# MichaelAxtmann/InPlaceMSDradixsort

Measured on AMD Instinct MI355X. Metric: Gkeys/s + achieved HBM GB/s, 2^30 uniform u32 keys, 1/2/4/8 MI355X, higher is better.
Workload: dtype u32; 1 GPU; 2^30 uniform u32 keys per GPU, in-place MSD radix sort, 8-bit digits; config_id=c2, elements_per_gpu=1073741824, steps_verified=0, verified_by=not checked in a plain run (bench.py --full verifies every timed step), workspace_bytes=360054784

## Files before the change

inplacemsdradixsort_amd/csrc/msd_device.hpp:

```cpp
#pragma once

#include <hip/hip_runtime.h>
#include <stdint.h>

namespace msd {

constexpr int kP = 256;
constexpr uint32_t kXBase = 0x80000000u;
constexpr uint32_t kNoOwner = 0xFFFFFFFFu;
constexpr uint32_t kRposStride = 32;

struct NoVal {};
typedef uint32_t u32x4 __attribute__((ext_vector_type(4)));

template <typename V> struct has_val { static constexpr bool value = true; };
template <> struct has_val<NoVal> { static constexpr bool value = false; };

template <typename K, typename V> struct Cfg;
template <> struct Cfg<uint32_t, NoVal> {
	static constexpr int B = 64, T = 4096, TH = 1024;
	static constexpr int SORT_TH = 1024, SORT_KPT = 24;
};
template <> struct Cfg<uint64_t, NoVal> {
	static constexpr int B = 32, T = 4096, TH = 1024;
// ... 317 lines not shown
	}
#pragma unroll
	for (int o = 32; o > 0; o >>= 1) {
		seen += (uint32_t)__shfl_xor((int)seen, o);
		same += (uint32_t)__shfl_xor((int)same, o);
	}
	if ((tid & 63) == 0 && seen) {
		atomicAdd(&plans[st.parent].adj_seen, seen);
		atomicAdd(&plans[st.parent].adj_same, same);
	}
}

#ifndef MSD_UNEVEN_PCT
#define MSD_UNEVEN_PCT 125
#endif
__device__ __forceinline__ bool direct_declines(uint32_t mn, uint32_t mx, uint32_t adj_same, uint32_t adj_seen)
{
	const bool runs = (uint64_t)adj_same * 8u > adj_seen;
	return runs || !(mn > 0 && (double)mx * 100.0 <= (double)MSD_UNEVEN_PCT * (double)mn);
}

template <int B>
__global__ __launch_bounds__(256) void direct_plan_kernel(const Parent *__restrict__ parents, DirectPlan *__restrict__ plans,
	Counters *__restrict__ ctr)
{
	__shared__ uint64_t tmp[8];
	__shared__ uint32_t s_mn, s_mx;
	const Parent pa = parents[blockIdx.x];
	DirectPlan *plan = plans + blockIdx.x;
	const uint32_t d = threadIdx.x;
	if (d == 0) {
		s_mn = 0xFFFFFFFFu;
		s_mx = 0;
	}
	const uint64_t s0 = (pa.start + B - 1) / B, s1 = (pa.start + pa.count) / B;
	uint64_t total;
	const uint64_t c = plan->est_cnt[d];
	const uint64_t ex = block_excl_scan256_64(c, tmp, total);
	const uint64_t ns = s1 > s0 ? s1 - s0 : 0;
	plan->bound[d] = (uint32_t)(s0 + (total ? ex * ns / total : (uint64_t)d * ns / kP));
	if (d == 0) plan->bound[kP] = (uint32_t)s1;
	if (d < (1u << pa.width)) {
		atomicMin(&s_mn, (uint32_t)c);
		atomicMax(&s_mx, (uint32_t)c);
	}
	__syncthreads();
	if (d == 0 && direct_declines(s_mn, s_mx, plan->adj_same, plan->adj_seen)) atomicAdd(&ctr->direct_uneven, 1u);
}

__device__ __forceinline__ bool wave_select_smallest(uint32_t v, bool elig, int need, uint64_t &mask_out)
{
	uint64_t cand = __ballot(elig), selm = 0;
	if ((int)__popcll(cand) > need) {
#pragma unroll
		for (int bit = 9; bit >= 0; --bit) {
			const uint64_t zeros = cand & ~__ballot((v >> bit) & 1u);
// ... 1950 lines not shown
```

inplacemsdradixsort_amd/csrc/msd_front16.hpp:

```cpp
#pragma once

namespace msd {

constexpr int kF16Th = 1024;
constexpr uint32_t kF16Words = 1u << 15;
constexpr size_t kF16Lds = (size_t)kF16Words * 4 + 64 * 4;
constexpr int kF16Loads = 8;

struct FrontSummary {
	uint32_t top[kP];
	unsigned long long v_or, v_and;
	uint32_t adj_seen, adj_same[2];
	uint32_t overflow;
	uint32_t uneven[2];
	uint32_t nroute[5];
	uint32_t hopeless;
};
static_assert(sizeof(FrontSummary) % 8 == 0, "the OR / AND words take 64-bit atomics");

__device__ __forceinline__ void front_clear(FrontSummary *__restrict__ sum)
{
	uint32_t *w = reinterpret_cast<uint32_t *>(sum);
	for (uint32_t i = threadIdx.x; i < sizeof(FrontSummary) / 4; i += blockDim.x) w[i] = 0;
	__syncthreads();
	if (threadIdx.x == 0) sum->v_and = ~0ull;
}
__global__ __launch_bounds__(256) void front_init_kernel(FrontSummary *__restrict__ sum) { front_clear(sum); }

constexpr int kFpRuns = 32;
template <typename K>
__global__ __launch_bounds__(1024) void front_probe_kernel(const K *__restrict__ keys, uint64_t n, uint32_t shift, FrontSummary *__restrict__ sum)
{
	__shared__ uint32_t h[kP], s_mn, s_mx, s_same;
	const uint32_t tid = threadIdx.x;
	if (tid < kP) h[tid] = 0;
	if (tid == 0) {
		s_mn = 0xFFFFFFFFu;
		s_mx = 0;
		s_same = 0;
// ... 133 lines not shown
{
	__shared__ uint32_t s_st[3], s_r[5];
	if (sum->hopeless) return;
	const uint32_t t = threadIdx.x, p = blockIdx.x * kP + t, sh = (p & 1u) * 16u;
	if (t == 0) {
		s_st[0] = 0xFFFFFFFFu;
		s_st[1] = 0;
		s_st[2] = 0;
	}
	if (t < 5) s_r[t] = 0;
	__syncthreads();
	const uint32_t *src = partials + (p >> 1);
	uint32_t c = 0;
#pragma unroll 8
	for (uint32_t w = 0; w < nparts; ++w) c += (src[(size_t)w * kF16Words] >> sh) & 0xFFFFu;
	hist[p] = c;
	atomicAdd(&s_r[(int)route_child(c, child_bits, stop_bits, count_bits, small_max, med_max, true) + 1], 1u);
	front_row_stats(c, s_st);
	if (t == 0) {
		sum->top[blockIdx.x] = s_st[2];
		if (direct_declines(s_st[0], s_st[1], sum->adj_same[1], sum->adj_seen)) atomicAdd(&sum->uneven[1], 1u);
	}
	if (t < 5 && s_r[t]) atomicAdd(&sum->nroute[t], s_r[t]);
}

__global__ __launch_bounds__(256) void front_top_kernel(FrontSummary *__restrict__ sum)
{
	__shared__ uint32_t s_st[3];
	if (sum->hopeless) return;
	if (threadIdx.x == 0) {
		s_st[0] = 0xFFFFFFFFu;
		s_st[1] = 0;
		s_st[2] = 0;
	}
	__syncthreads();
	front_row_stats(sum->top[threadIdx.x], s_st);
	if (threadIdx.x == 0 && direct_declines(s_st[0], s_st[1], sum->adj_same[0], sum->adj_seen)) sum->uneven[0] = 1;
}

__global__ __launch_bounds__(256) void front_apply_kernel(DirectPlan *__restrict__ plans, const uint32_t *__restrict__ hist,
	const FrontSummary *__restrict__ sum, uint32_t rows)
{
	DirectPlan *plan = plans + blockIdx.x;
	plan->est_cnt[threadIdx.x] = rows ? hist[blockIdx.x * kP + threadIdx.x] : sum->top[threadIdx.x];
	if (threadIdx.x == 0) {
		plan->adj_seen = sum->adj_seen;
		plan->adj_same = sum->adj_same[rows ? 1 : 0];
	}
}

}
```

inplacemsdradixsort_amd/csrc/msd_radix.hip:

```cpp
#include "msd_device.hpp"
#include "msd_select.hpp"
#include "msd_select_rows.hpp"
#include "msd_reverse.hpp"
#include "msd_sort_rows.hpp"
#include "msd_runs.hpp"
#include "msd_reduce.hpp"
#include "msd_scan.hpp"
#include "msd_compact.hpp"
#include "msd_search.hpp"
#include "msd_merge2.hpp"
#include "msd_setops.hpp"
#include "msd_join.hpp"
#include "msd_args.hpp"
#include "../../include/msd_radix_hip.h"
#include "../../include/msd_sort_keys_hip.h"
#include "../../include/msd_sort_rows_hip.h"
#include "../../include/msd_runs_hip.h"
#include "../../include/msd_reduce_hip.h"
#include "../../include/msd_scan_hip.h"
#include "../../include/msd_compact_hip.h"
#include "../../include/msd_search_hip.h"
#include "../../include/msd_merge_hip.h"
#include "../../include/msd_setops_hip.h"
#include "../../include/msd_join_hip.h"
// ... 8 lines not shown
#include <vector>

using namespace msd;

#define MSD_VERSION "inplacemsdradixsort_amd 0.2 (gfx950)"

struct PhaseRec {
	const char *name;
	hipEvent_t ev;
};

struct msd_ctx {
	int device = 0;
	hipStream_t stream = nullptr;
	char *slab = nullptr;
	size_t slab_bytes = 0;
	char *keep = nullptr;
	size_t keep_bytes = 0;
	Segment *lists = nullptr;
	size_t lists_cap = 0;
	void *pinned = nullptr;
	size_t pinned_bytes = 0;
	hipEvent_t ev_early = nullptr;
	std::string err;
	bool profiling = false;
	hipEvent_t ev_start = nullptr;
	std::vector<PhaseRec> phases;
	std::vector<hipEvent_t> ev_pool;
	size_t ev_used = 0;
	std::vector<std::pair<std::string, double>> phase_us;
	std::vector<std::pair<std::string, uint64_t>> stats;
	int sm_count = 256;
	int chains_per_cu[3] = { 4, 4, 2 };
	int direct_mode = 1;
	uint64_t direct_min = 1ull << 22;
	uint64_t direct_min_parent = 1ull << 17;
	int regpart = 1;
	int count16 = 1;
	int leaf17 = 1;
	int mid_leaf = 1;
	int early_leaves = 1;
	int early_plan = 1;
	int front_count = 1;
	uint64_t front_min = 1ull << 29;
	const uint32_t *order_keys = nullptr;
	uint64_t order_n = 0;
	int merge_leaf = 0;
	char *sel = nullptr;
	size_t sel_bytes = 0;
	uint64_t select_cap = 1ull << 20;
	int topk_rows_mode = 0;
	int topk_rows_lanes = 0;
	char *rows_stage = nullptr;
	size_t rows_stage_bytes = 0;
	int sort_rows_mode = 0;
	int sort_rows_lanes = 0;
	uint64_t *fix_plan = nullptr;
	int fix_stats = 0;
	uint64_t fix_split = 0;
	int search_mode = 0;
	uint64_t search_merge_ratio = 32;
};

static int fail(msd_ctx *c, int code, const char *fmt, ...)
{
	char buf[512];
	va_list ap;
// ... 419 lines not shown
template <typename K, typename V>
static size_t round_bytes_estimate(uint64_t n, int sm_count)
{
	using C = Cfg<K, V>;
	const uint64_t small_max = (uint64_t)C::SORT_TH * C::SORT_KPT;
	size_t worst = 0;
	for (int shape = 0; shape < 2; ++shape) {
		std::vector<Segment> segs;
		if (shape == 0)
			segs.push_back({ 0, n, (uint32_t)(sizeof(K) * 8), 0 });
		else if (n > 512 * small_max)
			for (int i = 0; i < 256; ++i) segs.push_back({ n / 256 * i, n / 256, (uint32_t)(sizeof(K) * 8 - 8), 0 });
		if (segs.empty()) continue;
		RoundPlan rp;
		plan_round<K, V>(segs, small_max, sm_count, rp);
		Bump b(nullptr);
		RoundBufs rb;
		carve_round<K, V>(b, rp, small_max, rb);
		worst = std::max(worst, b.off);
	}
	return worst + 4096;
}

template <typename K> struct SortJob {
	enum Kind {
		kWhole,
		kDigit,
		kRanges,
		kOffsets,
		kList,
	} kind = kWhole;
	uint32_t stop_bits = 0;
	unsigned shift = 0, width = 0;
	uint64_t *counts = nullptr;
	const K *splitters = nullptr;
	const uint64_t *seg_off = nullptr;
	uint32_t nsplit = 0, nseg = 0;
	const std::vector<Segment> *segs = nullptr;

	static SortJob whole(uint32_t stop_bits = 0) { return { kWhole, stop_bits }; }
	static SortJob digit(unsigned shift, unsigned width, uint64_t *counts) { return { kDigit, 0, shift, width, counts }; }
	static SortJob ranges(const K *delims, uint32_t nsplit, unsigned width, uint64_t *counts) { return { kRanges, 0, 0, width, counts, delims, nullptr, nsplit }; }
	static SortJob offsets(const uint64_t *seg_off, uint32_t nseg) { return { kOffsets, 0, 0, 0, nullptr, nullptr, seg_off, 0, nseg }; }
	static SortJob list(const std::vector<Segment> &segs) { return { kList, 0, 0, 0, nullptr, nullptr, nullptr, 0, 0, &segs }; }
	bool single_pass() const { return kind == kDigit || kind == kRanges; }
	bool segmented() const { return kind == kOffsets || kind == kList; }
// ... 101 lines not shown
			if (top_sample > 0 && c->direct_mode != 0 && n >= c->direct_min && n >= ((uint64_t)1 << 24)) {
				unverified = true;
				claimed_const = low_mask & ~(((uint64_t)1 << top_sample) - 1ull);
				cur[0].bits = (uint32_t)top_sample;
				set_stat(c, "skipped_bits", (uint64_t)(end_bit - top_sample));
			} else {
				rc = run_vary(1, &vary);
				if (rc) return rc;
				vary &= low_mask;
				const int top = vary ? 64 - __builtin_clzll(vary) : 0;
				set_stat(c, "skipped_bits", (uint64_t)(end_bit - top));
				if (top == 0)
					cur.clear();
				else
					cur[0].bits = (uint32_t)top;
			}
		}
		phase_mark(c, "bit skip");
		if (!cur.empty() && cur[0].bits <= job.stop_bits) cur.clear();
		return MSD_OK;
	}

	bool front = false;
	FrontSummary fsum;
	uint32_t *front_hist() const { return reinterpret_cast<uint32_t *>(c->lists + c->lists_cap); }
	FrontSummary *front_sum() const { return reinterpret_cast<FrontSummary *>(front_hist() + (size_t)kP * kP); }
	int front_count()
	{
		if constexpr (!HV && sizeof(K) == 4) {
			if (!c->front_count || job.kind != SortJob<K>::kWhole || job.stop_bits || end_bit != 32 || cur.size() != 1 || c->direct_mode == 0 ||
			    n < c->direct_min || n < c->front_min || n < ((uint64_t)1 << 20) || n >= ((uint64_t)1 << 32))
				return MSD_OK;
			{
				const uint64_t mean = n / kP;
				if (pick_width(n, 32, small_max, count_bits) != 8 || mean - mean / 8 < c->direct_min_parent ||
				    pick_width(mean - mean / 8, 24, small_max, count_bits) != 8 || pick_width(mean + mean / 8, 24, small_max, count_bits) != 8)
					return MSD_OK;
			}
			int rc = slab_reserve(c, round_bytes_estimate<K, V>(n, c->sm_count), true);
			if (!rc) rc = lists_reserve(c, (size_t)kP * kP + 16, 0, 0);
			if (rc) return rc;
			static_assert(((size_t)kP * kP + 16) * sizeof(Segment) >= (size_t)kP * kP * 4 + sizeof(FrontSummary), "the counts and the summary fit a quarter of the lists");
			const unsigned grid = (unsigned)std::min<uint64_t>({ (uint64_t)c->sm_count, std::max<uint64_t>(1, n >> 18), c->slab_bytes / (kF16Words * sizeof(uint32_t)) });
			if (!grid) return MSD_OK;
			uint32_t *partials = reinterpret_cast<uint32_t *>(c->slab);
			LAUNCH(c, (front_probe_kernel<K>), 1, 1024, 0, keys, n, 16u, front_sum());
			LAUNCH(c, (front_count16_kernel<K>), grid, kF16Th, kF16Lds, keys, n, 16u, partials, front_sum());
			LAUNCH(c, front_plan_kernel, kP, 256, 0, partials, grid, front_hist(), front_sum(), 16u, job.stop_bits, count_bits, small_max,
			       std::max<uint64_t>(small_max, kCountMedMax));
			LAUNCH(c, front_top_kernel, 1, 256, 0, front_sum());
			HIPCHK(c, hipMemcpyAsync(c->pinned, front_sum(), sizeof(FrontSummary), hipMemcpyDeviceToHost, c->stream));
			HIPCHK(c, hipStreamSynchronize(c->stream));
			memcpy(&fsum, c->pinned, sizeof fsum);
			phase_mark(c, "front count");
			const uint64_t vary = (fsum.v_or ^ fsum.v_and) & low_mask;
			const int top = vary ? 64 - __builtin_clzll(vary) : 0;
			if (fsum.hopeless) {
				add_stat(c, "front_count_declined", 1);
				return MSD_OK;
			}
			bool ok = !fsum.overflow && top + 8 > end_bit && !fsum.uneven[0] && !fsum.uneven[1] && fsum.nroute[kRouteCount + 1] == (uint32_t)kP * kP;
			std::vector<Segment> next = front_parents();
			uint64_t total = 0;
			for (const Segment &sg : next) {
				ok = ok && sg.count >= c->direct_min_parent && pick_width(sg.count, sg.bits, small_max, count_bits) == 8;
				total += sg.count;
			}
			if (!fsum.overflow && total != n) return fail(c, MSD_EINTERNAL, "front count: the counts add up to %llu of %llu keys", (unsigned long long)total, (unsigned long long)n);
			add_stat(c, ok ? "front_count_sorts" : "front_count_declined", 1);
			front = ok;
		}
		return MSD_OK;
	}
	std::vector<Segment> front_parents() const
	{
		std::vector<Segment> v;
		uint64_t at = 0;
		for (int d = 0; d < kP; ++d) {
			v.push_back({ at, fsum.top[d], (uint32_t)end_bit - 8u, 0 });
			at += fsum.top[d];
		}
		return v;
	}

	int route_to_leaves()
	{
		if (job.segmented() && !cur.empty()) {
			std::vector<Segment> l_small, l_count, l_big, parents;
			for (auto &sg : cur) {
				Route to = route_child(sg.count, sg.bits, job.stop_bits, HV ? 0u : count_bits, small_max, std::max<uint64_t>(small_max, kCountMedMax), !HV);
				if (to == kRouteDone) continue;
				if (to == kRouteBig && l_big.size() >= big_cap) to = kRouteNext;
// ... 32 lines not shown
		return MSD_OK;
	}

	int rounds()
	{
		while (!cur.empty() || dev_np) {
			int rc;
			if constexpr (sizeof(K) == 8) {
				if (!job.single_pass() && c->regpart) {
					std::vector<Segment> fit, rest;
					if (!dev_np)
						for (auto &sg : cur) (sg.count + 1 <= kRpCap && sg.count > small_max ? fit : rest).push_back(sg);
					if (dev_np || fit.size() >= 64 || (!fit.empty() && rest.empty())) {
						if constexpr (HV)
							rc = c->leaf17 && leaf17_ok && !unverified ? leaf17_pass(fit, rest) : regpart_round(fit, rest);
						else
							rc = regpart_round(fit, rest);
						if (rc) return rc;
						continue;
					}
				}
			}
			Round r;
			if ((rc = plan_upload(r)) || (rc = classify(r)) || (rc = permute_blocks(r)) || (rc = cleanup_collect(r)) ||
			    (rc = r.leaves_follow ? early_summary(r) : r.plan_ahead ? plan_next_early(r) : round_summary(r)))
				return rc;
		}
		return MSD_OK;
	}

	int leaf17_pass(const std::vector<Segment> &fit, const std::vector<Segment> &rest)
	{
		const bool on_device = dev_np != 0;
		const uint32_t np = on_device ? dev_np : (uint32_t)fit.size();
		dev_np = 0;
		int rc = slab_reserve(c, 2 * (size_t)np * sizeof(Segment) + 4096);
		if (!rc) rc = pinned_reserve(c, (size_t)np * sizeof(Segment) + 4096);
		if (rc) return rc;
		Segment *d_segs = reinterpret_cast<Segment *>(c->slab), *d_rej = d_segs + np;
		if (on_device)
			HIPCHK(c, hipMemcpyAsync(d_segs, dev_list, (size_t)np * sizeof(Segment), hipMemcpyDeviceToDevice, c->stream));
		else if ((rc = upload(c, { { d_segs, fit.data(), (size_t)np * sizeof(Segment) } })))
			return rc;
		HIPCHK(c, hipMemsetAsync(&ctr->nslow2, 0, sizeof(uint32_t), c->stream));
		HIPCHK(c, hipMemsetAsync(&ctr->l17_slow, 0, sizeof(uint32_t), c->stream));
		phase_mark(c, "plan+upload");
		LAUNCH(c, (leaf17_kernel<V>), std::min<uint32_t>(np, (uint32_t)c->sm_count), kL17Th, kL17Lds, keys, vals, d_segs, np, d_rej, &ctr->nslow2, ctr, 0);
// ... 63 lines not shown
		ncount_host = hc.ncount;
		nbig_host = hc.nbig;
		add_stat(c, "rounds", 1);
		add_stat(c, "regpart_rounds", 1);
		add_stat(c, "parents", np);
		add_stat(c, "children", nc);
		cur = rest;
		if (hc.next_parents && (rc = fetch_segments(c, d_next, hc.next_parents, cur, (char *)c->pinned + 256, ahead))) return rc;
		phase_mark(c, "readback");
		prev_direct = false;
		++round;
		return MSD_OK;
	}

	struct Round {
		RoundPlan rp;
		RoundBufs rb;
		uint32_t np = 0, ns = 0, nc = 0;
		bool tried_direct = false;
		bool hist_checks = false;
		bool leaves_follow = false;
		size_t plan_ahead = 0;
	};
	static constexpr size_t kReadAhead = 2048, kSegOff = 256, kVresOff = kSegOff - 2 * sizeof(unsigned long long);
	static constexpr size_t kEarlyOff = kSegOff + kReadAhead * sizeof(Segment), kStagingBytes = kEarlyOff + sizeof(Counters);
	static_assert(sizeof(Counters) <= kVresOff, "counters and the OR/AND words share the head of the staging buffer");
	static constexpr size_t kPlanCtrOff = (kStagingBytes + 255) / 256 * 256, kPlanSegOff = kPlanCtrOff + 256;
	static constexpr size_t kParkOff = kPlanSegOff + kReadAhead * sizeof(Segment), kStage2Off = (kParkOff + sizeof(Counters) + 255) / 256 * 256;
	static_assert(sizeof(Counters) <= 256, "the early copy of the counters has 256 bytes");
	struct Pending {
		bool open = false;
		int round = 0;
		uint32_t np = 0, ns = 0, nc = 0;
		uint64_t nslots = 0;
	} pending;
	Pending parked;
	bool parked_direct = false;
	bool enqueue_ahead = false;
	Counters *park() const { return ctr + 2; }
	static size_t stage2_bytes(size_t np, size_t ns) { return kStage2Off + np * sizeof(Parent) + ns * sizeof(Stripe); }
	void plan_next(const std::vector<Segment> &segs, RoundPlan &rp) const
	{
		plan_round<K, V>(segs, small_max, c->sm_count, rp, count_bits, job.single_pass() ? job.width : 0u, job.splitters ? job.nsplit : 0u);
	}
	int plan_upload(Round &r)
	{
		const bool ahead = enqueue_ahead;
		enqueue_ahead = false;
		plan_next(cur, r.rp);
		const bool first = round == 0;
		int rc = slab_carve(c, [&](Bump &b) { carve_round<K, V>(b, r.rp, small_max, r.rb); },
				    first && !job.single_pass() ? round_bytes_estimate<K, V>(n, c->sm_count) : 0, first);
		if (rc) return rc;
		r.np = (uint32_t)r.rp.parents.size(), r.ns = (uint32_t)r.rp.stripes.size(), r.nc = r.rp.nchildren;
		if constexpr (!HV) {
			r.leaves_follow = !job.single_pass() && !unverified && c->early_leaves;
			for (size_t i = 0; i < r.np && r.leaves_follow; ++i) r.leaves_follow = r.rp.parents[i].shift <= count_bits;
		}
		if ((rc = lists_reserve(c, (size_t)std::max(nsmall_host, ncount_host) + r.nc + 16, nsmall_host, ncount_host))) return rc;
		{
			static_assert(sizeof(Parent) % 4 == 0 && sizeof(Stripe) % 4 == 0, "the plan travels as 32-bit words");
			const uint64_t plan_words = (r.np <= kDirectMaxParents ? r.np : 1) * sizeof(DirectPlan) / sizeof(uint32_t);
			const uint64_t ntiles = (r.nc + kScanTile - 1) / kScanTile + 1;
			const uint64_t parent_words = r.np * sizeof(Parent) / 4, stripe_words = r.ns * sizeof(Stripe) / 4;
			const size_t next_stripes = (size_t)std::max<uint64_t>((uint64_t)c->sm_count * MSD_STRIPE_WANT, n >> MSD_STRIPE_CAP_LOG) + 2 * kReadAhead + 64;
			const size_t want = !ahead && c->early_plan && !job.single_pass() ? stage2_bytes(kReadAhead, next_stripes) : 0;
			if ((rc = pinned_reserve(c, std::max({ kStagingBytes, r.np * sizeof(Parent) + r.ns * sizeof(Stripe), want })))) return rc;
			char *stage = (char *)c->pinned + (ahead ? kStage2Off : 0);
			if (!ahead) HIPCHK(c, hipStreamSynchronize(c->stream));
			memcpy(stage, r.rp.parents.data(), r.np * sizeof(Parent));
			memcpy(stage + r.np * sizeof(Parent), r.rp.stripes.data(), r.ns * sizeof(Stripe));
			void *staged = nullptr;
			HIPCHK(c, hipHostGetDevicePointer(&staged, c->pinned, 0));
			staged = (char *)staged + (stage - (char *)c->pinned);
			const unsigned grid = (unsigned)std::min<uint64_t>(1024, (std::max({ plan_words, ntiles, parent_words, stripe_words }) + 255) / 256 + 1);
			LAUNCH(c, round_init_kernel, grid, 256, 0, ctr, reinterpret_cast<uint32_t *>(r.rb.plans), plan_words, r.rb.scan_state, ntiles, r.rb.scan_ctr,
			       static_cast<const uint32_t *>(staged), reinterpret_cast<uint32_t *>(r.rb.parents), parent_words,
			       reinterpret_cast<uint32_t *>(r.rb.stripes), stripe_words, ahead ? park() : nullptr);
		}
		phase_mark(c, "plan+upload");
		return MSD_OK;
	}

	int classify_direct(Round &r)
	{
		const RoundPlan &rp = r.rp;
		const uint32_t np = r.np, ns = r.ns;
		bool try_direct = c->direct_mode != 0 && rp.round_keys >= c->direct_min && !job.splitters;
		for (size_t i = 0; i < np && try_direct; ++i) try_direct = rp.parents[i].width == 8 || c->direct_mode == 2;
		if (try_direct && np > 1) {
			try_direct = prev_direct && np <= kDirectMaxParents;
			for (size_t i = 0; i < np && try_direct; ++i) try_direct = rp.parents[i].count >= c->direct_min_parent;
		}
		for (size_t i = 0; i < ns && try_direct; ++i)
			try_direct = rp.stripes[i].end - rp.stripes[i].begin >= (((uint64_t)1 << rp.parents[rp.stripes[i].parent].width) * (B - 1) + 2 * B);
		uint64_t max_piece = 0;
		for (size_t i = 0; i < np && try_direct; ++i)
			max_piece = std::max<uint64_t>(max_piece, rp.parents[i].count / B / (rp.parents[i].stripe_hi - rp.parents[i].stripe_lo) + 2);
		if (front && (round > 1 || np != (round == 0 ? 1u : (uint32_t)kP))) front = false;
		if (!try_direct || max_piece >= 65535) {
			front = false;
			return MSD_OK;
		}
		const RoundBufs &rb = r.rb;
		if (front) {
			LAUNCH(c, front_apply_kernel, np, 256, 0, rb.plans, front_hist(), front_sum(), (uint32_t)round);
		} else if (np == 1) {
			const uint64_t nruns = rp.parents[0].count / 256;
			const uint32_t every = (uint32_t)std::min<uint64_t>(64, std::max<uint64_t>(1, nruns / 16384));
			const uint32_t sgrid = (uint32_t)std::min<uint64_t>(1024, std::max<uint64_t>(1, nruns / every / 4));
			LAUNCH(c, (direct_sample_kernel<K>), sgrid, 256, 0, keys, rb.parents, rb.plans, every);
		} else {
			r.hist_checks = unverified && rp.round_keys == n;
			if (r.hist_checks) {
				if (int rc = vres_init()) return rc;
				add_stat(c, "bit_skip_checked_by_histogram", 1);
			}
			LAUNCH(c, (direct_hist_kernel<K>), ns, 1024, 0, keys, rb.stripes, rb.parents, rb.plans, r.hist_checks ? vres : nullptr);
		}
		LAUNCH(c, (direct_plan_kernel<B>), np, 256, 0, rb.parents, rb.plans, ctr);
		phase_mark(c, front ? "A front counts" : np == 1 ? "A sample" : "A histogram");
		r.tried_direct = true;
		const uint32_t force = c->direct_mode == 2 ? 1u : 0u;
		LAUNCH(c, (classify_direct2_kernel<K, V>), ns, (Direct2Cfg<K, V>::TH), (Direct2Lds<K, V>::bytes), keys, vals, rb.stripes, rb.parents, rb.plans,
		       block_map, slot_full, rb.fb, rb.lo_cnt, rb.lo_off, rb.lo_keys, rb.lo_vals, rb.nfull, ctr, force);
		phase_mark(c, "A classify direct");
		return MSD_OK;
	}

	int classify(Round &r)
	{
		if (int rc = classify_direct(r)) return rc;
		if (!r.tried_direct || c->direct_mode != 2) {
			const RoundBufs &rb = r.rb;
			const uint32_t *run_if = r.tried_direct ? &ctr->direct_uneven : nullptr;
			if (job.splitters)
				LAUNCH(c, (classify_stream2_kernel<K, V, true>), r.ns, (Stream2Cfg<K, V>::TH), (Stream2Lds<K, V>::range_bytes), keys, vals, rb.stripes,
				       rb.parents, block_map, rb.fb, rb.lo_cnt, rb.lo_off, rb.lo_keys, rb.lo_vals, rb.nfull, job.splitters, run_if);
			else
				LAUNCH(c, (classify_stream2_kernel<K, V, false>), r.ns, (Stream2Cfg<K, V>::TH), (Stream2Lds<K, V>::bytes), keys, vals, rb.stripes,
				       rb.parents, block_map, rb.fb, rb.lo_cnt, rb.lo_off, rb.lo_keys, rb.lo_vals, rb.nfull, nullptr, run_if);
		}
		phase_mark(c, "A classify");
// ... 30 lines not shown
		LAUNCH(c, (chains_kernel<K, V>), grid, 256, 0, rb.ca, rb.list, rb.holes, ctr, keys, vals, rb.xkeys, rb.xvals, n / B, 4 * nc + kMinChains);
		phase_mark(c, "B block permute");
		return MSD_OK;
	}

	bool may_leave_parents(const Round &r) const
	{
		uint64_t leaf_max = small_max;
		if constexpr (sizeof(K) == 8)
			if (c->regpart) leaf_max = std::max<uint64_t>(leaf_max, kRpCap - 1);
		for (const Parent &p : r.rp.parents)
			if ((p.count >> p.width) > leaf_max) return true;
		return false;
	}

	int collect(Round &r)
	{
		const RoundBufs &rb = r.rb;
		const uint32_t np = r.np, nc = r.nc;
		const bool sp = job.single_pass();
		uint32_t wmax = 1;
		for (size_t i = 0; i < np; ++i) wmax = std::max(wmax, r.rp.parents[i].width);
		const uint32_t small_cap = (uint32_t)std::min<size_t>(c->lists_cap, 0xFFFFFFFFu);
		LAUNCH(c, collect_kernel, (np + (256u >> wmax) - 1) / (256u >> wmax), 256, 0, rb.parents, np, wmax, rb.ca,
		       sp ? ~0ull : small_max, (HV || sp) ? small_max : std::max<uint64_t>(small_max, kCountMedMax),
		       small_cap, sp ? 0u : count_bits,
		       rb.next_parents, small(), small_count(), (HV || sp) ? nullptr : big, big_cap, ctr,
		       (sp && job.counts) ? job.counts : nullptr, job.splitters ? job.nsplit + 1u : nc, job.stop_bits);
		if (r.leaves_follow) {
			if (front && round == 1) return MSD_OK;
			if (!c->ev_early) HIPCHK(c, hipEventCreateWithFlags(&c->ev_early, hipEventDisableTiming));
			HIPCHK(c, hipMemcpyAsync((char *)c->pinned + kEarlyOff, ctr, sizeof(Counters), hipMemcpyDeviceToHost, c->stream));
			HIPCHK(c, hipEventRecord(c->ev_early, c->stream));
		} else if (c->early_plan && !sp && !r.hist_checks && !parked.open && c->pinned_bytes >= kStage2Off && may_leave_parents(r)) {
			r.plan_ahead = std::min<size_t>(r.rp.round_keys / (small_max + 1) + 2, kReadAhead);
			if (front && round == 0) return MSD_OK;
			if (!c->ev_early) HIPCHK(c, hipEventCreateWithFlags(&c->ev_early, hipEventDisableTiming));
			HIPCHK(c, hipMemcpyAsync((char *)c->pinned + kPlanCtrOff, ctr, sizeof(Counters), hipMemcpyDeviceToHost, c->stream));
			HIPCHK(c, hipMemcpyAsync((char *)c->pinned + kPlanSegOff, rb.next_parents, r.plan_ahead * sizeof(Segment), hipMemcpyDeviceToHost, c->stream));
			HIPCHK(c, hipEventRecord(c->ev_early, c->stream));
		}
		return MSD_OK;
	}

	int cleanup_collect(Round &r)
	{
		const RoundBufs &rb = r.rb;
// ... 124 lines not shown
			if ((h[0] ^ h[1]) & claimed_const) {
				exact_vary = h[0] ^ h[1];
				phase_mark(c, "readback");
				return kRestart;
			}
			unverified = false;
		}
		prev_direct = r.tried_direct && (hc.direct_uneven == 0 || c->direct_mode == 2);
		if (prev_direct) add_stat(c, "direct_rounds", 1);
		nsmall_host = hc.nsmall;
		ncount_host = hc.ncount;
		nbig_host = hc.nbig;
		round_stats(hc, r.np, r.ns, r.nc, r.rp.nslots);
		cur.clear();
		if (job.single_pass()) return MSD_OK;
		bool stays_on_device = false;
		if constexpr (sizeof(K) == 8) {
			if (c->regpart && hc.next_parents >= 64 && (uint64_t)hc.next_max + 1 <= kRpCap) {
				HIPCHK(c, hipMemcpyAsync(dev_list, r.rb.next_parents, (size_t)hc.next_parents * sizeof(Segment), hipMemcpyDeviceToDevice, c->stream));
				dev_np = hc.next_parents;
				stays_on_device = true;
			}
		}
		if (hc.next_parents && !stays_on_device &&
		    (rc = fetch_segments(c, r.rb.next_parents, hc.next_parents, cur, (char *)c->pinned + kSegOff, ahead)))
			return rc;
		phase_mark(c, "readback");
		++round;
		return MSD_OK;
	}

	int verify_skip()
	{
		if (!unverified) return MSD_OK;
		uint64_t vary = 0;
		if (int rc = run_vary(1, &vary)) return rc;
		phase_mark(c, "bit skip");
		if (vary & claimed_const) {
			exact_vary = vary;
			return kRestart;
		}
		unverified = false;
		return MSD_OK;
	}

	int start_over()
	{
		const uint64_t vary = exact_vary & low_mask;
		const int top = vary ? 64 - __builtin_clzll(vary) : 0;
		set_stat(c, "skipped_bits", (uint64_t)(end_bit - top));
		add_stat(c, "bit_skip_restarts", 1);
		cur.clear();
		if (top > 0 && (uint32_t)top > job.stop_bits) cur.push_back({ 0, n, (uint32_t)top, 0 });
		nsmall_host = ncount_host = nbig_host = dev_np = 0;
		round = 0;
		pending.open = parked.open = enqueue_ahead = false;
		prev_direct = unverified = front = false;
		HIPCHK(c, hipMemsetAsync(ctr, 0, sizeof(Counters), c->stream));
		return MSD_OK;
	}

	int count_leaves()
	{
		if constexpr (!HV) {
			if (!ncount_host || job.single_pass()) return MSD_OK;
			int rc = slab_reserve(c, 3 * (size_t)ncount_host * sizeof(Segment) + 4096);
			if (rc) return rc;
			Segment *slow = reinterpret_cast<Segment *>(c->slab), *rej16 = slow + ncount_host, *slow2 = rej16 + ncount_host;
			const uint32_t count_grid = std::min<uint32_t>(ncount_host, (uint32_t)c->sm_count * 2);
			const bool c16 = sizeof(K) == 4 && (c->count16 == 2 || (c->count16 == 1 && n / ncount_host >= 12000));
			if constexpr (sizeof(K) == 4)
				if (c16) LAUNCH(c, count_place16_kernel, count_grid, kC16Th, kC16Lds, keys, small_count(), ncount_host, rej16, ctr, n);
			LAUNCH(c, (count_place_kernel<K>), count_grid, kCountTh, kCountLds, keys, c16 ? rej16 : small_count(), c16 ? 0u : ncount_host,
			       c16 ? &ctr->nslow16 : nullptr, slow, ctr);
			const uint32_t *walk_n = &ctr->nslow;
			const Segment *walk_list = slow;
			if constexpr (sizeof(K) == 4) {
				if (c->mid_leaf) {
					LAUNCH(c, (merge_count_kernel<true>), std::min<uint32_t>(ncount_host, (uint32_t)c->sm_count), kMcTh, kMcLds, keys, keys, nullptr,
					       nullptr, nullptr, 0, 0, 0, 0, slow, &ctr->nslow, slow2, &ctr->nslow2, &ctr->count_ticket4, nullptr);
					walk_n = &ctr->nslow2;
					walk_list = slow2;
				}
			}
			LAUNCH(c, (count_walk_kernel<K>), count_grid, kCountTh, kCountLds, keys, walk_list, walk_n, small(), nsmall_host, small_max, big, big_cap, ctr);
			phase_mark(c, "count sort");
			Counters hc;
			if ((rc = read_counters(c, ctr, hc, { parked_piece() })) || (rc = parked_summary())) return rc;
			if (pending.open) {
				pending.open = false;
				if (hc.errors && (hc.err_sites & ~0x80u || !hc.err_sites))
					return round_errors(hc, pending.round, pending.np, pending.ns, prev_direct ? "used" : "not used");
				round_stats(hc, pending.np, pending.ns, pending.nc, pending.nslots);
			}
			if (hc.errors) return fail(c, MSD_EINTERNAL, "counting leaf: %u segments could not be queued", hc.errors);
			set_stat(c, "count16_rejected", hc.nslow16);
			set_stat(c, "count_slow_segments", hc.nslow);
			nbig_host = hc.nbig;
			nfallback_known = hc.nfallback;
		}
		return MSD_OK;
	}

	int big_count_sort()
	{
		if constexpr (!HV) {
			if (!nbig_host || job.single_pass()) return MSD_OK;
			std::vector<Segment> bs;
			int rc = fetch(c, big, nbig_host, bs);
			if (rc) return rc;
			const uint32_t batch_max = 4096;
			for (uint32_t b0 = 0; b0 < nbig_host; b0 += batch_max) {
				const uint32_t nb = std::min(batch_max, nbig_host - b0);
				constexpr uint32_t tile_elems = big_tile_elems<K>() * kBigGroup;
				std::vector<uint32_t> first(2 * ((size_t)nb + 1));
				uint32_t *first_chunk = first.data(), *first_tile = first.data() + nb + 1;
				uint64_t nchunks = 0, ntiles = 0;
				for (uint32_t i = 0; i < nb; ++i) {
					first_chunk[i] = (uint32_t)nchunks;
					first_tile[i] = (uint32_t)ntiles;
					nchunks += (bs[b0 + i].count + kBigChunk - 1) / kBigChunk;
					ntiles += (bs[b0 + i].count + tile_elems - 1) / tile_elems;
				}
// ... 60 lines not shown
		return MSD_OK;
	}
};

}

template <typename K, typename V>
static int sort_impl(msd_ctx *c, K *keys, uint64_t *vals, uint64_t n, int end_bit, const SortJob<K> &job)
{
	constexpr bool HV = has_val<V>::value;
	if (n == 0) return MSD_OK;
	if (!keys || (HV && !vals)) return fail(c, MSD_EINVAL, "null data pointer");
	if (!aligned16(keys) || (HV && !aligned16(vals)))
		return fail(c, MSD_EINVAL, "keys/rids must be 16-byte aligned (the reference asserts the same, src/msb_64.c:2273)");
	if (end_bit < 0 || end_bit > (int)sizeof(K) * 8) return fail(c, MSD_EINVAL, "end_bit out of range");
	if (n >= ((uint64_t)1 << 36)) return fail(c, MSD_EINVAL, "n too large for 32-bit block slots");
	HIPCHK(c, hipSetDevice(c->device));
	c->stats.clear();
	phase_begin(c);
	SortRun<K, V> s(c, keys, vals, n, end_bit, job);
	int rc = s.initial_segments();
	if (!rc) rc = s.reserve_keep();
	if (!rc) rc = s.front_count();
	if (!rc && !s.front) rc = s.skip_leading_bits();
	if (!rc) rc = s.route_to_leaves();
	while (!rc) {
		rc = s.rounds();
		if (!rc) rc = s.verify_skip();
		if (rc != kRestart) break;
		rc = s.start_over();
	}
	if (!rc) rc = s.count_leaves();
	if (!rc) rc = s.big_count_sort();
	if (rc) return rc;
	set_stat(c, "big_count_segments", s.nbig_host);
	if ((rc = s.lds_leaves())) return rc;
	set_stat(c, "count_segments", s.ncount_host);
	set_stat(c, "small_segments", s.nsmall_host);
	set_stat(c, "workspace_bytes", c->slab_bytes + c->keep_bytes + 4 * c->lists_cap * sizeof(Segment));
	phase_end(c);
	return MSD_OK;
}

template <typename K, typename V> static int reserve_for(msd_ctx *c, uint64_t n)
{
	int rc = slab_reserve(c, round_bytes_estimate<K, V>(n, c->sm_count), true);
	if (!rc) rc = keep_reserve(c, keep_bytes_for<K, V>(n), true);
	if (!rc) rc = pinned_reserve(c, 1 << 20);
	if (!rc) rc = lists_reserve(c, leaf_list_guess<K, V>(n), 0, 0, true);
	return rc;
}

constexpr int kNoLayout = 1;
template <typename F> static int with_layout(int key_bytes, int val_bytes, F &&f)
{
	if (key_bytes == 4 && val_bytes == 0) return f(uint32_t(), NoVal());
	if (key_bytes == 8 && val_bytes == 0) return f(uint64_t(), NoVal());
	if (key_bytes == 8 && val_bytes == 8) return f(uint64_t(), uint64_t());
	return kNoLayout;
}

template <typename K, typename V> static int sort_bits(msd_ctx *c, K *k, uint64_t *r, uint64_t n, int end_bit)
{
	if (!c) return MSD_EINVAL;
	return sort_impl<K, V>(c, k, r, n, end_bit, SortJob<K>::whole());
}
template <typename K, typename V> static int partition(msd_ctx *c, K *k, uint64_t *r, uint64_t n, unsigned shift, unsigned rb, uint64_t *cnt)
{
	if (!c) return MSD_EINVAL;
// ... 157 lines not shown
	if (rc) {
		fprintf(stderr, "msd_create: %s\n", c->err.c_str());
		delete c;
		return rc;
	}
	*out = c;
	return MSD_OK;
}

int msd_destroy(msd_ctx *c)
{
	if (!c) return MSD_EINVAL;
	(void)hipSetDevice(c->device);
	(void)hipStreamSynchronize(c->stream);
	if (c->slab) (void)hipFree(c->slab);
	if (c->keep) (void)hipFree(c->keep);
	if (c->lists) (void)hipFree(c->lists);
	if (c->sel) (void)hipFree(c->sel);
	if (c->rows_stage) (void)hipFree(c->rows_stage);
	if (c->fix_plan) (void)hipFree(c->fix_plan);
	if (c->pinned) (void)hipHostFree(c->pinned);
	if (c->ev_start) (void)hipEventDestroy(c->ev_start);
	if (c->ev_early) (void)hipEventDestroy(c->ev_early);
	for (auto e : c->ev_pool) (void)hipEventDestroy(e);
	delete c;
	return MSD_OK;
}

int msd_set_stream(msd_ctx *c, void *stream)
{
	if (!c) return MSD_EINVAL;
	c->stream = (hipStream_t)stream;
	return MSD_OK;
}

void *msd_get_stream(const msd_ctx *c) { return c ? (void *)c->stream : nullptr; }
int msd_get_device(const msd_ctx *c) { return c ? c->device : -1; }

int msd_reserve(msd_ctx *c, uint64_t n, int key_bytes, int val_bytes)
{
	if (!c) return MSD_EINVAL;
	HIPCHK(c, hipSetDevice(c->device));
	const int rc = with_layout(key_bytes, val_bytes, [&](auto k, auto v) { return reserve_for<decltype(k), decltype(v)>(c, n); });
	return rc != kNoLayout ? rc : fail(c, MSD_EINVAL, "unsupported element layout %d+%d bytes", key_bytes, val_bytes);
}

// ... 1638 lines not shown
{
	if (!c || !name) return MSD_EINVAL;
	if (!strcmp(name, "direct_mode")) {
		if (value < 0 || value > 2) return fail(c, MSD_EINVAL, "direct_mode must be 0, 1 or 2");
		c->direct_mode = (int)value;
	} else if (!strcmp(name, "direct_min")) {
		if (value < 1) return fail(c, MSD_EINVAL, "direct_min must be positive");
		c->direct_min = (uint64_t)value;
	} else if (!strcmp(name, "regpart")) {
		c->regpart = value != 0;
	} else if (!strcmp(name, "count16")) {
		if (value < 0 || value > 2) return fail(c, MSD_EINVAL, "count16 must be 0, 1 or 2");
		c->count16 = (int)value;
	} else if (!strcmp(name, "leaf17")) {
		c->leaf17 = value != 0;
	} else if (!strcmp(name, "mid_leaf")) {
		c->mid_leaf = value != 0;
	} else if (!strcmp(name, "early_leaves")) {
		c->early_leaves = value != 0;
	} else if (!strcmp(name, "early_plan")) {
		c->early_plan = value != 0;
	} else if (!strcmp(name, "front_count")) {
		c->front_count = value != 0;
	} else if (!strcmp(name, "front_min")) {
		if (value < 1) return fail(c, MSD_EINVAL, "front_min must be positive");
		c->front_min = (uint64_t)value;
	} else if (!strcmp(name, "merge_leaf")) {
		if (value < 0 || value > 2) return fail(c, MSD_EINVAL, "merge_leaf must be 0, 1 or 2");
		c->merge_leaf = (int)value;
	} else if (!strcmp(name, "select_cap")) {
		if (value < 1 || value > ((int64_t)1 << 28)) return fail(c, MSD_EINVAL, "select_cap must be 1 .. 2^28 elements");
		c->select_cap = (uint64_t)value;
	} else if (!strcmp(name, "topk_rows_mode")) {
		if (value < 0 || value > 2) return fail(c, MSD_EINVAL, "topk_rows_mode must be 0, 1 or 2");
		c->topk_rows_mode = (int)value;
	} else if (!strcmp(name, "topk_rows_lanes")) {
		if (value != 0 && value != 64 && value != 256 && value != 1024) return fail(c, MSD_EINVAL, "topk_rows_lanes must be 0, 64, 256 or 1024");
		c->topk_rows_lanes = (int)value;
	} else if (!strcmp(name, "sort_rows_mode")) {
		if (value < 0 || value > 2) return fail(c, MSD_EINVAL, "sort_rows_mode must be 0, 1 or 2");
		c->sort_rows_mode = (int)value;
	} else if (!strcmp(name, "sort_rows_lanes")) {
		if (value != 0 && value != 64 && value != 256 && value != 1024) return fail(c, MSD_EINVAL, "sort_rows_lanes must be 0, 64, 256 or 1024");
		c->sort_rows_lanes = (int)value;
	} else if (!strcmp(name, "search_mode")) {
		if (value < 0 || value > 2) return fail(c, MSD_EINVAL, "search_mode must be 0, 1 or 2");
// ... 56 lines not shown
```

Baseline: 157.3 Gkeys/s.

## Enqueue round 0 speculatively behind front count, gated by a device-side verdict

Folds the front_top step into the last block of front_plan_kernel, which computes a device-side go flag. The host then plans and enqueues round 0's classification before waiting on the front summary, and direct_plan_kernel reads the front counts directly, so front_apply_kernel is removed. If the host's verdict disagrees, the speculative round is dropped. Also caches the round-bytes estimate, skips the collect kernel on round 0, and adds an early exit in the count-sort leaf when no second stage is needed. The aim is to hide the host sync and planning latency behind GPU work, at the cost of a more complex control flow and a consistency check between host and device verdicts.

Result: faster. 158.9 Gkeys/s (median of 6 runs) (+1.0%).

```diff
diff --git a/inplacemsdradixsort_amd/csrc/msd_device.hpp b/inplacemsdradixsort_amd/csrc/msd_device.hpp
--- a/inplacemsdradixsort_amd/csrc/msd_device.hpp
+++ b/inplacemsdradixsort_amd/csrc/msd_device.hpp
@@ -363,16 +363,27 @@
 
 template <int B>
 __global__ __launch_bounds__(256) void direct_plan_kernel(const Parent *__restrict__ parents, DirectPlan *__restrict__ plans,
-	Counters *__restrict__ ctr)
+	Counters *__restrict__ ctr, const uint32_t *front_cnt, const uint32_t *adj_seen, const uint32_t *adj_same, const uint32_t *go)
 {
 	__shared__ uint64_t tmp[8];
 	__shared__ uint32_t s_mn, s_mx;
+	const uint32_t d = threadIdx.x;
+	if (go && !*go) {
+		if (d == 0) atomicAdd(&ctr->direct_uneven, 1u);
+		return;
+	}
 	const Parent pa = parents[blockIdx.x];
 	DirectPlan *plan = plans + blockIdx.x;
-	const uint32_t d = threadIdx.x;
 	if (d == 0) {
 		s_mn = 0xFFFFFFFFu;
 		s_mx = 0;
+	}
+	if (front_cnt) {
+		plan->est_cnt[d] = front_cnt[blockIdx.x * kP + d];
+		if (d == 0) {
+			plan->adj_seen = *adj_seen;
+			plan->adj_same = *adj_same;
+		}
 	}
 	const uint64_t s0 = (pa.start + B - 1) / B, s1 = (pa.start + pa.count) / B;
 	uint64_t total;
diff --git a/inplacemsdradixsort_amd/csrc/msd_front16.hpp b/inplacemsdradixsort_amd/csrc/msd_front16.hpp
--- a/inplacemsdradixsort_amd/csrc/msd_front16.hpp
+++ b/inplacemsdradixsort_amd/csrc/msd_front16.hpp
@@ -15,6 +15,8 @@
 	uint32_t uneven[2];
 	uint32_t nroute[5];
 	uint32_t hopeless;
+	uint32_t done;
+	uint32_t go;
 };
 static_assert(sizeof(FrontSummary) % 8 == 0, "the OR / AND words take 64-bit atomics");
 
@@ -194,31 +196,24 @@
 		if (direct_declines(s_st[0], s_st[1], sum->adj_same[1], sum->adj_seen)) atomicAdd(&sum->uneven[1], 1u);
 	}
 	if (t < 5 && s_r[t]) atomicAdd(&sum->nroute[t], s_r[t]);
-}
-
-__global__ __launch_bounds__(256) void front_top_kernel(FrontSummary *__restrict__ sum)
-{
-	__shared__ uint32_t s_st[3];
-	if (sum->hopeless) return;
-	if (threadIdx.x == 0) {
+	__shared__ uint32_t s_last;
+	if (t == 0) s_last = __hip_atomic_fetch_add(&sum->done, 1u, __ATOMIC_ACQ_REL, __HIP_MEMORY_SCOPE_AGENT) == gridDim.x - 1 ? 1u : 0u;
+	__syncthreads();
+	if (!s_last) return;
+	__threadfence();
+	if (t == 0) {
 		s_st[0] = 0xFFFFFFFFu;
 		s_st[1] = 0;
 		s_st[2] = 0;
 	}
 	__syncthreads();
-	front_row_stats(sum->top[threadIdx.x], s_st);
-	if (threadIdx.x == 0 && direct_declines(s_st[0], s_st[1], sum->adj_same[0], sum->adj_seen)) sum->uneven[0] = 1;
-}
-
-__global__ __launch_bounds__(256) void front_apply_kernel(DirectPlan *__restrict__ plans, const uint32_t *__restrict__ hist,
-	const FrontSummary *__restrict__ sum, uint32_t rows)
-{
-	DirectPlan *plan = plans + blockIdx.x;
-	plan->est_cnt[threadIdx.x] = rows ? hist[blockIdx.x * kP + threadIdx.x] : sum->top[threadIdx.x];
-	if (threadIdx.x == 0) {
-		plan->adj_seen = sum->adj_seen;
-		plan->adj_same = sum->adj_same[rows ? 1 : 0];
-	}
-}
-
-}
+	front_row_stats(__hip_atomic_load(&sum->top[t], __ATOMIC_RELAXED, __HIP_MEMORY_SCOPE_AGENT), s_st);
+	if (t == 0) {
+		const bool uneven = direct_declines(s_st[0], s_st[1], sum->adj_same[0], sum->adj_seen);
+		const bool top_varies = (((sum->v_or ^ sum->v_and) >> (child_bits + 8u)) & 0xFFull) != 0;
+		if (uneven) sum->uneven[0] = 1;
+		sum->go = (!uneven && top_varies && !sum->overflow) ? 1u : 0u;
+	}
+}
+
+}
diff --git a/inplacemsdradixsort_amd/csrc/msd_radix.hip b/inplacemsdradixsort_amd/csrc/msd_radix.hip
--- a/inplacemsdradixsort_amd/csrc/msd_radix.hip
+++ b/inplacemsdradixsort_amd/csrc/msd_radix.hip
@@ -54,6 +54,7 @@
 	void *pinned = nullptr;
 	size_t pinned_bytes = 0;
 	hipEvent_t ev_early = nullptr;
+	hipEvent_t ev_front = nullptr;
 	std::string err;
 	bool profiling = false;
 	hipEvent_t ev_start = nullptr;
@@ -74,7 +75,11 @@
 	int early_leaves = 1;
 	int early_plan = 1;
 	int front_count = 1;
+	int front_ahead = 1;
 	uint64_t front_min = 1ull << 29;
+	uint64_t est_n = 0;
+	int est_layout = -1, est_cus = 0;
+	size_t est_bytes = 0;
 	const uint32_t *order_keys = nullptr;
 	uint64_t order_n = 0;
 	int merge_leaf = 0;
@@ -540,6 +545,18 @@
 	return worst + 4096;
 }
 
+template <typename K, typename V> static size_t round_bytes_cached(msd_ctx *c, uint64_t n)
+{
+	const int layout = (int)sizeof(K) * 2 + (has_val<V>::value ? 1 : 0);
+	if (c->est_layout != layout || c->est_n != n || c->est_cus != c->sm_count) {
+		c->est_bytes = round_bytes_estimate<K, V>(n, c->sm_count);
+		c->est_layout = layout;
+		c->est_n = n;
+		c->est_cus = c->sm_count;
+	}
+	return c->est_bytes;
+}
+
 template <typename K> struct SortJob {
 	enum Kind {
 		kWhole,
@@ -687,6 +704,7 @@
 	}
 
 	bool front = false;
+	bool front_gated = false;
 	FrontSummary fsum;
 	uint32_t *front_hist() const { return reinterpret_cast<uint32_t *>(c->lists + c->lists_cap); }
 	FrontSummary *front_sum() const { return reinterpret_cast<FrontSummary *>(front_hist() + (size_t)kP * kP); }
@@ -702,8 +720,12 @@
 				    pick_width(mean - mean / 8, 24, small_max, count_bits) != 8 || pick_width(mean + mean / 8, 24, small_max, count_bits) != 8)
 					return MSD_OK;
 			}
-			int rc = slab_reserve(c, round_bytes_estimate<K, V>(n, c->sm_count), true);
+			int rc = slab_reserve(c, round_bytes_cached<K, V>(c, n), true);
 			if (!rc) rc = lists_reserve(c, (size_t)kP * kP + 16, 0, 0);
+			const bool ahead = c->front_ahead && c->direct_mode != 2;
+			if (!rc && ahead)
+				rc = pinned_reserve(c, std::max({ kStagingBytes, kFrontStageOff + sizeof(Parent) + next_stripes_max() * sizeof(Stripe),
+								  c->early_plan ? stage2_bytes(kReadAhead, next_stripes_max()) : 0 }));
 			if (rc) return rc;
 			static_assert(((size_t)kP * kP + 16) * sizeof(Segment) >= (size_t)kP * kP * 4 + sizeof(FrontSummary), "the counts and the summary fit a quarter of the lists");
 			const unsigned grid = (unsigned)std::min<uint64_t>({ (uint64_t)c->sm_count, std::max<uint64_t>(1, n >> 18), c->slab_bytes / (kF16Words * sizeof(uint32_t)) });
@@ -713,16 +735,36 @@
 			LAUNCH(c, (front_count16_kernel<K>), grid, kF16Th, kF16Lds, keys, n, 16u, partials, front_sum());
 			LAUNCH(c, front_plan_kernel, kP, 256, 0, partials, grid, front_hist(), front_sum(), 16u, job.stop_bits, count_bits, small_max,
 			       std::max<uint64_t>(small_max, kCountMedMax));
-			LAUNCH(c, front_top_kernel, 1, 256, 0, front_sum());
 			HIPCHK(c, hipMemcpyAsync(c->pinned, front_sum(), sizeof(FrontSummary), hipMemcpyDeviceToHost, c->stream));
-			HIPCHK(c, hipStreamSynchronize(c->stream));
+			phase_mark(c, "front count");
+			bool enqueued = false;
+			if (ahead) {
+				if (!c->ev_front) HIPCHK(c, hipEventCreateWithFlags(&c->ev_front, hipEventDisableTiming));
+				HIPCHK(c, hipEventRecord(c->ev_front, c->stream));
+				front = front_gated = true;
+				rc = plan_upload(ahead_r);
+				if (!rc) rc = classify_direct(ahead_r);
+				front = front_gated = false;
+				if (rc) return rc;
+				phase_mark(c, "A classify");
+				enqueued = ahead_r.tried_direct;
+				HIPCHK(c, hipEventSynchronize(c->ev_front));
+			} else
+				HIPCHK(c, hipStreamSynchronize(c->stream));
 			memcpy(&fsum, c->pinned, sizeof fsum);
-			phase_mark(c, "front count");
 			const uint64_t vary = (fsum.v_or ^ fsum.v_and) & low_mask;
 			const int top = vary ? 64 - __builtin_clzll(vary) : 0;
+			const auto drop = [&]() -> int {
+				ahead_r = Round();
+				if (ahead) HIPCHK(c, hipMemsetAsync(ctr, 0, sizeof(Counters), c->stream));
+				if (enqueued) add_stat(c, "front_ahead_dropped", 1);
+				return MSD_OK;
+			};
+			if (enqueued && (fsum.go != 0) != (!fsum.hopeless && !fsum.overflow && top + 8 > end_bit && !fsum.uneven[0]))
+				return fail(c, MSD_EINTERNAL, "front count: the device's verdict on round 0 (%u) is not the summary's", fsum.go);
 			if (fsum.hopeless) {
 				add_stat(c, "front_count_declined", 1);
-				return MSD_OK;
+				return drop();
 			}
 			bool ok = !fsum.overflow && top + 8 > end_bit && !fsum.uneven[0] && !fsum.uneven[1] && fsum.nroute[kRouteCount + 1] == (uint32_t)kP * kP;
 			std::vector<Segment> next = front_parents();
@@ -733,6 +775,11 @@
 			}
 			if (!fsum.overflow && total != n) return fail(c, MSD_EINTERNAL, "front count: the counts add up to %llu of %llu keys", (unsigned long long)total, (unsigned long long)n);
 			add_stat(c, ok ? "front_count_sorts" : "front_count_declined", 1);
+			if (enqueued && fsum.go) {
+				ahead_live = true;
+				add_stat(c, "front_ahead_kept", 1);
+			} else if ((rc = drop()))
+				return rc;
 			front = ok;
 		}
 		return MSD_OK;
@@ -811,7 +858,13 @@
 				}
 			}
 			Round r;
-			if ((rc = plan_upload(r)) || (rc = classify(r)) || (rc = permute_blocks(r)) || (rc = cleanup_collect(r)) ||
+			if (ahead_live) {
+				ahead_live = false;
+				r = std::move(ahead_r);
+				rc = MSD_OK;
+			} else if (!(rc = plan_upload(r)))
+				rc = classify(r);
+			if (rc || (rc = permute_blocks(r)) || (rc = cleanup_collect(r)) ||
 			    (rc = r.leaves_follow ? early_summary(r) : r.plan_ahead ? plan_next_early(r) : round_summary(r)))
 				return rc;
 		}
@@ -921,6 +974,8 @@
 		bool leaves_follow = false;
 		size_t plan_ahead = 0;
 	};
+	Round ahead_r;
+	bool ahead_live = false;
 	static constexpr size_t kReadAhead = 2048, kSegOff = 256, kVresOff = kSegOff - 2 * sizeof(unsigned long long);
 	static constexpr size_t kEarlyOff = kSegOff + kReadAhead * sizeof(Segment), kStagingBytes = kEarlyOff + sizeof(Counters);
 	static_assert(sizeof(Counters) <= kVresOff, "counters and the OR/AND words share the head of the staging buffer");
@@ -938,6 +993,12 @@
 	bool enqueue_ahead = false;
 	Counters *park() const { return ctr + 2; }
 	static size_t stage2_bytes(size_t np, size_t ns) { return kStage2Off + np * sizeof(Parent) + ns * sizeof(Stripe); }
+	static constexpr size_t kFrontStageOff = 2048;
+	static_assert(sizeof(FrontSummary) <= kFrontStageOff, "the summary lands in front of round 0's staged plan");
+	size_t next_stripes_max() const
+	{
+		return (size_t)std::max<uint64_t>((uint64_t)c->sm_count * MSD_STRIPE_WANT, n >> MSD_STRIPE_CAP_LOG) + 2 * kReadAhead + 64;
+	}
 	void plan_next(const std::vector<Segment> &segs, RoundPlan &rp) const
 	{
 		plan_round<K, V>(segs, small_max, c->sm_count, rp, count_bits, job.single_pass() ? job.width : 0u, job.splitters ? job.nsplit : 0u);
@@ -945,11 +1006,20 @@
 	int plan_upload(Round &r)
 	{
 		const bool ahead = enqueue_ahead;
+		const bool gated = front_gated;
 		enqueue_ahead = false;
 		plan_next(cur, r.rp);
+		if (gated) {
+			Bump sz(nullptr);
+			RoundBufs probe;
+			carve_round<K, V>(sz, r.rp, small_max, probe);
+			if (sz.off + 4096 > c->slab_bytes || (size_t)r.rp.nchildren + 16 > c->lists_cap ||
+			    kFrontStageOff + r.rp.parents.size() * sizeof(Parent) + r.rp.stripes.size() * sizeof(Stripe) > c->pinned_bytes)
+				return fail(c, MSD_EINTERNAL, "front count: round 0 does not fit the workspace reserved for it");
+		}
 		const bool first = round == 0;
 		int rc = slab_carve(c, [&](Bump &b) { carve_round<K, V>(b, r.rp, small_max, r.rb); },
-				    first && !job.single_pass() ? round_bytes_estimate<K, V>(n, c->sm_count) : 0, first);
+				    first && !job.single_pass() ? round_bytes_cached<K, V>(c, n) : 0, first);
 		if (rc) return rc;
 		r.np = (uint32_t)r.rp.parents.size(), r.ns = (uint32_t)r.rp.stripes.size(), r.nc = r.rp.nchildren;
 		if constexpr (!HV) {
@@ -962,11 +1032,10 @@
 			const uint64_t plan_words = (r.np <= kDirectMaxParents ? r.np : 1) * sizeof(DirectPlan) / sizeof(uint32_t);
 			const uint64_t ntiles = (r.nc + kScanTile - 1) / kScanTile + 1;
 			const uint64_t parent_words = r.np * sizeof(Parent) / 4, stripe_words = r.ns * sizeof(Stripe) / 4;
-			const size_t next_stripes = (size_t)std::max<uint64_t>((uint64_t)c->sm_count * MSD_STRIPE_WANT, n >> MSD_STRIPE_CAP_LOG) + 2 * kReadAhead + 64;
-			const size_t want = !ahead && c->early_plan && !job.single_pass() ? stage2_bytes(kReadAhead, next_stripes) : 0;
-			if ((rc = pinned_reserve(c, std::max({ kStagingBytes, r.np * sizeof(Parent) + r.ns * sizeof(Stripe), want })))) return rc;
-			char *stage = (char *)c->pinned + (ahead ? kStage2Off : 0);
-			if (!ahead) HIPCHK(c, hipStreamSynchronize(c->stream));
+			const size_t want = !ahead && c->early_plan && !job.single_pass() ? stage2_bytes(kReadAhead, next_stripes_max()) : 0;
+			if (!gated && (rc = pinned_reserve(c, std::max({ kStagingBytes, r.np * sizeof(Parent) + r.ns * sizeof(Stripe), want })))) return rc;
+			char *stage = (char *)c->pinned + (gated ? kFrontStageOff : ahead ? kStage2Off : 0);
+			if (!ahead && !gated) HIPCHK(c, hipStreamSynchronize(c->stream));
 			memcpy(stage, r.rp.parents.data(), r.np * sizeof(Parent));
 			memcpy(stage + r.np * sizeof(Parent), r.rp.stripes.data(), r.ns * sizeof(Stripe));
 			void *staged = nullptr;
@@ -1003,7 +1072,6 @@
 		}
 		const RoundBufs &rb = r.rb;
 		if (front) {
-			LAUNCH(c, front_apply_kernel, np, 256, 0, rb.plans, front_hist(), front_sum(), (uint32_t)round);
 		} else if (np == 1) {
 			const uint64_t nruns = rp.parents[0].count / 256;
 			const uint32_t every = (uint32_t)std::min<uint64_t>(64, std::max<uint64_t>(1, nruns / 16384));
@@ -1017,7 +1085,9 @@
 			}
 			LAUNCH(c, (direct_hist_kernel<K>), ns, 1024, 0, keys, rb.stripes, rb.parents, rb.plans, r.hist_checks ? vres : nullptr);
 		}
-		LAUNCH(c, (direct_plan_kernel<B>), np, 256, 0, rb.parents, rb.plans, ctr);
+		FrontSummary *const fs = front ? front_sum() : nullptr;
+		LAUNCH(c, (direct_plan_kernel<B>), np, 256, 0, rb.parents, rb.plans, ctr, fs ? (round == 0 ? fs->top : front_hist()) : nullptr,
+		       fs ? &fs->adj_seen : nullptr, fs ? &fs->adj_same[round == 0 ? 0 : 1] : nullptr, fs && front_gated ? &fs->go : nullptr);
 		phase_mark(c, front ? "A front counts" : np == 1 ? "A sample" : "A histogram");
 		r.tried_direct = true;
 		const uint32_t force = c->direct_mode == 2 ? 1u : 0u;
@@ -1094,7 +1164,8 @@
 		uint32_t wmax = 1;
 		for (size_t i = 0; i < np; ++i) wmax = std::max(wmax, r.rp.parents[i].width);
 		const uint32_t small_cap = (uint32_t)std::min<size_t>(c->lists_cap, 0xFFFFFFFFu);
-		LAUNCH(c, collect_kernel, (np + (256u >> wmax) - 1) / (256u >> wmax), 256, 0, rb.parents, np, wmax, rb.ca,
+		if (!(front && round == 0))
+			LAUNCH(c, collect_kernel, (np + (256u >> wmax) - 1) / (256u >> wmax), 256, 0, rb.parents, np, wmax, rb.ca,
 		       sp ? ~0ull : small_max, (HV || sp) ? small_max : std::max<uint64_t>(small_max, kCountMedMax),
 		       small_cap, sp ? 0u : count_bits,
 		       rb.next_parents, small(), small_count(), (HV || sp) ? nullptr : big, big_cap, ctr,
@@ -1265,8 +1336,10 @@
 				stays_on_device = true;
 			}
 		}
-		if (hc.next_parents && !stays_on_device &&
-		    (rc = fetch_segments(c, r.rb.next_parents, hc.next_parents, cur, (char *)c->pinned + kSegOff, ahead)))
+		if (front && round == 0)
+			cur = front_parents();
+		else if (hc.next_parents && !stays_on_device &&
+			 (rc = fetch_segments(c, r.rb.next_parents, hc.next_parents, cur, (char *)c->pinned + kSegOff, ahead)))
 			return rc;
 		phase_mark(c, "readback");
 		++round;
@@ -1298,7 +1371,7 @@
 		nsmall_host = ncount_host = nbig_host = dev_np = 0;
 		round = 0;
 		pending.open = parked.open = enqueue_ahead = false;
-		prev_direct = unverified = front = false;
+		prev_direct = unverified = front = ahead_live = false;
 		HIPCHK(c, hipMemsetAsync(ctr, 0, sizeof(Counters), c->stream));
 		return MSD_OK;
 	}
@@ -1314,6 +1387,14 @@
 			const bool c16 = sizeof(K) == 4 && (c->count16 == 2 || (c->count16 == 1 && n / ncount_host >= 12000));
 			if constexpr (sizeof(K) == 4)
 				if (c16) LAUNCH(c, count_place16_kernel, count_grid, kC16Th, kC16Lds, keys, small_count(), ncount_host, rej16, ctr, n);
+			const bool on_demand = front && c16;
+			Counters hc;
+			if (on_demand) {
+				phase_mark(c, "count sort");
+				if ((rc = leaf_counters(hc))) return rc;
+				set_stat(c, "count_second_stage", hc.nslow16 ? 1 : 0);
+				if (!hc.nslow16) return leaf_stats(hc);
+			}
 			LAUNCH(c, (count_place_kernel<K>), count_grid, kCountTh, kCountLds, keys, c16 ? rej16 : small_count(), c16 ? 0u : ncount_host,
 			       c16 ? &ctr->nslow16 : nullptr, slow, ctr);
 			const uint32_t *walk_n = &ctr->nslow;
@@ -1328,20 +1409,30 @@
 			}
 			LAUNCH(c, (count_walk_kernel<K>), count_grid, kCountTh, kCountLds, keys, walk_list, walk_n, small(), nsmall_host, small_max, big, big_cap, ctr);
 			phase_mark(c, "count sort");
-			Counters hc;
-			if ((rc = read_counters(c, ctr, hc, { parked_piece() })) || (rc = parked_summary())) return rc;
-			if (pending.open) {
-				pending.open = false;
-				if (hc.errors && (hc.err_sites & ~0x80u || !hc.err_sites))
-					return round_errors(hc, pending.round, pending.np, pending.ns, prev_direct ? "used" : "not used");
-				round_stats(hc, pending.np, pending.ns, pending.nc, pending.nslots);
-			}
-			if (hc.errors) return fail(c, MSD_EINTERNAL, "counting leaf: %u segments could not be queued", hc.errors);
-			set_stat(c, "count16_rejected", hc.nslow16);
-			set_stat(c, "count_slow_segments", hc.nslow);
-			nbig_host = hc.nbig;
-			nfallback_known = hc.nfallback;
-		}
+			if ((rc = leaf_counters(hc))) return rc;
+			return leaf_stats(hc);
+		}
+		return MSD_OK;
+	}
+	int leaf_counters(Counters &hc)
+	{
+		int rc;
+		if ((rc = read_counters(c, ctr, hc, { parked_piece() })) || (rc = parked_summary())) return rc;
+		if (pending.open) {
+			pending.open = false;
+			if (hc.errors && (hc.err_sites & ~0x80u || !hc.err_sites))
+				return round_errors(hc, pending.round, pending.np, pending.ns, prev_direct ? "used" : "not used");
+			round_stats(hc, pending.np, pending.ns, pending.nc, pending.nslots);
+		}
+		if (hc.errors) return fail(c, MSD_EINTERNAL, "counting leaf: %u segments could not be queued", hc.errors);
+		return MSD_OK;
+	}
+	int leaf_stats(const Counters &hc)
+	{
+		set_stat(c, "count16_rejected", hc.nslow16);
+		set_stat(c, "count_slow_segments", hc.nslow);
+		nbig_host = hc.nbig;
+		nfallback_known = hc.nfallback;
 		return MSD_OK;
 	}
 
@@ -1448,7 +1539,7 @@
 	int rc = s.initial_segments();
 	if (!rc) rc = s.reserve_keep();
 	if (!rc) rc = s.front_count();
-	if (!rc && !s.front) rc = s.skip_leading_bits();
+	if (!rc && !s.front && !s.ahead_live) rc = s.skip_leading_bits();
 	if (!rc) rc = s.route_to_leaves();
 	while (!rc) {
 		rc = s.rounds();
@@ -1470,7 +1561,7 @@
 
 template <typename K, typename V> static int reserve_for(msd_ctx *c, uint64_t n)
 {
-	int rc = slab_reserve(c, round_bytes_estimate<K, V>(n, c->sm_count), true);
+	int rc = slab_reserve(c, round_bytes_cached<K, V>(c, n), true);
 	if (!rc) rc = keep_reserve(c, keep_bytes_for<K, V>(n), true);
 	if (!rc) rc = pinned_reserve(c, 1 << 20);
 	if (!rc) rc = lists_reserve(c, leaf_list_guess<K, V>(n), 0, 0, true);
@@ -1674,6 +1765,7 @@
 	if (c->pinned) (void)hipHostFree(c->pinned);
 	if (c->ev_start) (void)hipEventDestroy(c->ev_start);
 	if (c->ev_early) (void)hipEventDestroy(c->ev_early);
+	if (c->ev_front) (void)hipEventDestroy(c->ev_front);
 	for (auto e : c->ev_pool) (void)hipEventDestroy(e);
 	delete c;
 	return MSD_OK;
@@ -3358,6 +3450,8 @@
 		c->early_plan = value != 0;
 	} else if (!strcmp(name, "front_count")) {
 		c->front_count = value != 0;
+	} else if (!strcmp(name, "front_ahead")) {
+		c->front_ahead = value != 0;
 	} else if (!strcmp(name, "front_min")) {
 		if (value < 1) return fail(c, MSD_EINVAL, "front_min must be positive");
 		c->front_min = (uint64_t)value;
```
